# ikramanop/aligner

Hardware: AMD Instinct MI355X
Metric: GCUPS (DP cell updates/s), fill + traceback, inputs resident in HBM (higher is better)
Workload: dtype int32; 1 GPU; C5: 100000 protein pairs, lengths iid U[200,2000], core local (SimpleLocalAligner), BLOSUM62, del 11 / ext 2, seed 0xA11C0005; pairs=100000, cells=121325988939, pairs_ok_rank0=100000, pairs_repaired_or_refilled_rank0=65570

## Files before the change

### aligner_amd/csrc/aln_device.h

```cpp
#pragma once
#include <stdint.h>

#include "../../include/aligner_hip.h"

#ifndef ALN_FULL_R
#define ALN_FULL_R 8
#endif
#define ALN_STRIP_ROWS (64 * ALN_FULL_R)
#define ALN_LAYOUT_SKEW 0u
#define ALN_LAYOUT_ROWMAJOR 1u
#define ALN_LAYOUT_UNIFORM 2u
#define ALN_LAYOUT_UBATCH 3u

struct PairDesc {
    uint64_t q_off, t_off;
    uint32_t N, M;
    uint64_t dir_off;
    uint64_t tb_off;
    uint64_t tag_off;
    uint64_t h_off;
    int32_t status;
    uint32_t layout;
};
#define ALN_PRE_EMPTY_OK (-1)
// ... 85 lines not shown
#define ALN_COOP_ABORTS 6
#define ALN_COOP_SCANS 7
#define ALN_COOP_ULOG 32
#define ALN_COOP_CTL_WORDS 256u

struct SingleArgs {
    const uint8_t *seqs;
    PairDesc *descs;
    uint32_t pair;
    uint8_t *dirs;
    aln_pair_result *results;
    uint32_t *granules;
    uint64_t gstride;
    uint8_t *advice, *zrow;
    int32_t *cand;
    uint32_t *ctrl;
    const void *matrix;
    uint32_t rows, cols;
    double del, ext;
    int32_t semantics;
    uint32_t R, ns, pass, max_passes;
    uint32_t hazard;
    uint32_t store_dirs;
    uint32_t test_drop;
    int *ckpt;
    uint32_t *rgranules;
    int32_t *rcand;
    uint32_t rep_S, rep_K;
    uint32_t mode;
};

#define ALN_CK_SLOTS 7
#define ALN_CK_LAST 1024u
#define ALN_CASCADE_ROWS 3u
#define ALN_CK_FIRST 16u

struct TraceArgs {
    const uint8_t *seqs;
    const PairDesc *descs;
    uint32_t n_pairs;
    const uint8_t *dirs;
    aln_pair_result *results;
    uint8_t *tb;
    uint8_t *tags;
    int32_t semantics;
    uint8_t blank;
    uint8_t pwm;
    uint32_t *walked;
    uint32_t epoch;
    const uint32_t *doneq;
    uint32_t *head;
    uint32_t n_order;
    uint64_t wait_ticks;
};

struct WgArgs {
    const uint8_t *seqs;
    PairDesc *descs;
    uint32_t pair;
    uint8_t *dirs;
    aln_pair_result *results;
    const void *matrix;
    uint32_t rows, cols;
    double del, ext;
    int32_t semantics;
    uint32_t R, ns;
    uint32_t max_passes;
    uint32_t store_dirs;
    uint8_t *scratch;
    void *hmat;
    uint32_t pwm;
};
#define ALN_WG_RING 256u
__host__ __device__ inline uint32_t aln_wg_lds_bytes(uint32_t rows, uint32_t cols, uint32_t sc_size, uint32_t ns, uint32_t N)
{
    return ((rows * cols * sc_size + 15u) & ~15u) + ns * ALN_WG_RING * sc_size + 3u * ((N + 66u + 15u) & ~15u) + 64u * 4u + ns * 32u +
           (N <= 2048u ? (((N + 66u) * sc_size + 15u) & ~15u) : 0u);
}
#define ALN_QRING_BYTES 192u
#define ALN_BRING_BYTES 272u
#define ALN_FEED_BYTES (ALN_QRING_BYTES + ALN_BRING_BYTES)
__host__ __device__ inline uint32_t aln_fast_lds_bytes(uint32_t rows, uint32_t cols, uint32_t prof_stride, uint32_t feed_bytes)
{
    const uint32_t s_bytes = (rows * cols * 4u + 15u) & ~15u;
    return prof_stride == 0u ? s_bytes : s_bytes + 4u * prof_stride + 4u * feed_bytes;
}

struct TraceSingleArgs {
    const uint8_t *seqs;
    const PairDesc *descs;
    uint32_t pair;
    const uint8_t *dirs;
    aln_pair_result *results;
    uint8_t *tb;
    uint8_t *tags;
    int32_t semantics;
    uint32_t R, ns;
    uint4 *map;
    uint4 *seg;
    uint32_t pwm;
};

__host__ __device__ constexpr inline uint32_t aln_spb(uint32_t R) { return R >= 5 ? 2u : R >= 3 ? 4u : 16u / R; }
__host__ __device__ inline int aln_tag_to_dir(int t) { return t == 3 ? 3 : 2 - t; }
__host__ __device__ inline int aln_dir_to_tag(int d) { return d == 3 ? 3 : 2 - d; }
__host__ __device__ inline uint32_t aln_dir_bitpos(uint32_t k, uint32_t r, uint32_t lane, uint32_t N, int R)
// ... 42 lines not shown
```

### aligner_amd/csrc/aln_host.hip

```cpp
#include <hip/hip_runtime.h>

#include <algorithm>
#include <atomic>
#include <cmath>
#include <condition_variable>
#include <cstdio>
#include <cstdlib>
#include <cstring>
#include <deque>
#include <memory>
#include <mutex>
#include <numeric>
#include <string>
#include <chrono>
#include <thread>
#include <vector>

#include "aln_device.h"
#include "aln_loop_rules.h"
#include "aln_plan_rules.h"
#include "aln_scheme_rules.h"
#include "aln_seqset_rules.h"
#include "aln_shuffle_rules.h"

// ... 40 lines not shown
    template <class T> T *as() const { return reinterpret_cast<T *>(p); }
};
static int dev_ensure(DevBuf &b, size_t bytes, bool slack)
{
    bytes = std::max<size_t>(bytes, 256);
    if (b.cap >= bytes) return ALN_OK;
    if (b.p) { (void)hipFree(b.p); b.p = nullptr; b.cap = 0; }
    size_t want = slack ? bytes + bytes / 8 : bytes;
    hipError_t e = hipMalloc(&b.p, want);
    if (e != hipSuccess && want != bytes) { want = bytes; e = hipMalloc(&b.p, want); }
    if (e != hipSuccess) { b.p = nullptr; return fail(e, "hipMalloc"); }
    b.cap = want;
    return ALN_OK;
}
static void dev_free(DevBuf &b)
{
    if (b.p) (void)hipFree(b.p);
    b.p = nullptr; b.cap = 0;
}
struct PinBuf {
    void *p = nullptr;
    size_t cap = 0;
    template <class T> T *as() const { return reinterpret_cast<T *>(p); }
};
static int pin_ensure(PinBuf &b, size_t bytes)
{
    bytes = std::max<size_t>(bytes, 4096);
    if (b.cap >= bytes) return ALN_OK;
    if (b.p) { (void)hipHostFree(b.p); b.p = nullptr; b.cap = 0; }
    const size_t want = bytes + bytes / 4;
    hipError_t e = hipHostMalloc(&b.p, want, hipHostMallocDefault);
    if (e != hipSuccess) { b.p = nullptr; return fail(e, "hipHostMalloc"); }
    b.cap = want;
    return ALN_OK;
}
static void pin_free(PinBuf &b)
{
    if (b.p) (void)hipHostFree(b.p);
    b.p = nullptr; b.cap = 0;
}

struct Slot {
    bool pooled = true;
    DevBuf seqs, descs, order, counter, walked, dirs, results, tb, tags, scratch, matrix, pwm_words, hmat;
    DevBuf granules, advice1, cand, ctrl, tbmap, unpack, repair, coop;
    DevBuf shuffle;
    PinBuf h_meta;
    PinBuf h_in, h_out;
    hipStream_t stream = nullptr;
    hipStream_t tb_stream = nullptr;
    hipEvent_t ev_fork = nullptr, ev_join = nullptr, ev_done = nullptr, ev_fill = nullptr;
    uint32_t epoch = 0;
    bool walked_clean = false;
    uint32_t salt = 0;
    bool scratch_clean = false;
};

struct DevCtx {
    int device = 0;
    int cus = 0;
    size_t hbm = 0;
    char name[128] = {0};
    std::mutex mu;
    std::condition_variable cv;
    Slot *slots[ALN_POOL_SLOTS] = {nullptr};
    bool busy[ALN_POOL_SLOTS] = {false};
};

struct aln_ctx {
    std::vector<DevCtx *> devs;
    std::atomic<uint32_t> turn{0};
    DevCtx *next_device() { return devs[turn.fetch_add(1, std::memory_order_relaxed) % devs.size()]; }
};

static int slot_init(Slot &s)
{
    if (!s.stream) HIPCHK(hipStreamCreateWithFlags(&s.stream, hipStreamNonBlocking));
    if (!s.ev_done) HIPCHK(hipEventCreateWithFlags(&s.ev_done, hipEventDisableTiming));
    if (!s.ev_fill) HIPCHK(hipEventCreateWithFlags(&s.ev_fill, hipEventDisableTiming));
    return ALN_OK;
}
static void slot_destroy(Slot *s)
{
    if (!s) return;
    DevBuf *d[] = {&s->seqs, &s->descs, &s->order, &s->counter, &s->walked, &s->dirs, &s->results, &s->tb, &s->tags, &s->scratch,
                   &s->matrix, &s->pwm_words, &s->hmat, &s->granules, &s->advice1, &s->cand, &s->ctrl, &s->tbmap, &s->unpack, &s->repair, &s->coop,
                   &s->shuffle};
    for (DevBuf *b : d) dev_free(*b);
    pin_free(s->h_meta); pin_free(s->h_in); pin_free(s->h_out);
    if (s->ev_fork) (void)hipEventDestroy(s->ev_fork);
    if (s->ev_join) (void)hipEventDestroy(s->ev_join);
    if (s->ev_done) (void)hipEventDestroy(s->ev_done);
    if (s->ev_fill) (void)hipEventDestroy(s->ev_fill);
    if (s->tb_stream) (void)hipStreamDestroy(s->tb_stream);
    if (s->stream) (void)hipStreamDestroy(s->stream);
    delete s;
}

static int pool_lease(DevCtx *ctx, int want, Slot **out)
{
    std::unique_lock<std::mutex> lk(ctx->mu);
    int got = 0;
    for (;;) {
        for (int i = 0; i < ALN_POOL_SLOTS && got < want; ++i)
            if (!ctx->busy[i]) {
                if (!ctx->slots[i]) ctx->slots[i] = new Slot();
// ... 454 lines not shown
    const uint64_t adv_bytes = ((uint64_t)max_len + 66 + 63) & ~63ull;
    k.cascade_rows = (c.fast && c.semantics == ALN_CORE_LOCAL && c.p.del != c.p.ext) ? ALN_CASCADE_ROWS : (c.fast ? 2u : 1u);
    const uint64_t ck_bytes = c.fast ? (uint64_t)ALN_CK_SLOTS * 18 * 64 * 4 : 0;
    const uint64_t zrow_bytes = std::max<uint64_t>(adv_bytes, ((c.fast ? 8ull : 4ull) * (((uint64_t)max_len + 63) / 2 + 8) + 63) & ~63ull);
    k.zrow_bytes = (uint32_t)zrow_bytes;
    const uint64_t row1_bytes = c.fast ? 0 : brow_bytes + adv_bytes;
    k.scratch_stride = (uint64_t)k.cascade_rows * brow_bytes + adv_bytes + zrow_bytes + ck_bytes + row1_bytes;
    k.lds_bytes = c.pair_matrices ? aln_pairset_lds_bytes(rows, cols) : (uint32_t)(((uint64_t)rows * cols * (c.is_int ? 4 : 8) + 15) & ~15ull);
    k.prof_stride = 0;
    if (c.fast && !pwm) { k.prof_stride = cols * 64u * ALN_FULL_R; k.lds_bytes = aln_fast_lds_bytes(rows, cols, k.prof_stride, ALN_FEED_BYTES); }
    k.duo_qo = 0;
    if (c.fast && !pwm && c.semantics == ALN_CORE_GLOBAL && !k.coop && !k.coop_lean && !k.overlap && !getenv("ALN_NO_DUO") &&
        k.n_small > (uint64_t)ctx->cus * 12u) {
        uint32_t max_rows = 0, max_cols = 0;
        for (size_t j = 0; j < k.n_small; ++j) { const PairDesc &d = k.descs[k.order[j]]; max_rows = std::max(max_rows, d.M); max_cols = std::max(max_cols, d.N); }
        const uint32_t qo = (max_cols + 136u + 7u) & ~7u;
        const uint32_t rmax = (max_rows + 31u) / 32u, rp = rmax > 4u ? 8u : rmax > 2u ? 4u : std::max(rmax, 1u);
        const uint32_t prof = cols * 64u * rp;
        const uint32_t lds = (uint32_t)(((uint64_t)rows * cols * 4 + 15) & ~15ull) + 4u * (prof + 4u * qo);
        if (max_rows <= 256u && max_cols <= 1024u && lds <= 52u * 1024u) {
            k.duo_qo = qo;
            k.prof_stride = prof;
            k.lds_bytes = lds;
            const uint32_t items = (uint32_t)((k.n_small + 1) / 2);
            k.grid = std::max(1u, std::min((items + 3u) / 4u, (uint32_t)ctx->cus * 3u));
        }
    }
    return ALN_OK;
}

struct Need {
    uint64_t seq_span = 0, n = 0, dir_bytes = 0, tb_bytes = 0, tag_bytes = 0, scratch = 0, coop = 0;
};

static int slot_ensure(Slot &s, const Call &c, const Chunk &k, const Need *need = nullptr, bool small_meta = false)
{
    int st;
    const bool sl = s.pooled;
#define ENS(buf, bytes) if ((st = dev_ensure(s.buf, (bytes), sl)) != ALN_OK) return st
    if (need) {
        ENS(seqs, need->seq_span + 64);
        ENS(descs, need->n * sizeof(PairDesc));
        ENS(order, need->n * sizeof(uint32_t));
        ENS(results, need->n * sizeof(aln_pair_result));
        ENS(dirs, need->dir_bytes);
        ENS(tb, need->tb_bytes);
        ENS(tags, need->tag_bytes);
        ENS(scratch, need->scratch);
        if (need->coop) ENS(coop, need->coop);
    }
    ENS(seqs, k.seq_span + 64);
    ENS(descs, k.n * sizeof(PairDesc));
    ENS(order, k.n * sizeof(uint32_t));
    ENS(counter, k.counter_bytes);
    if (k.coop) ENS(coop, k.coop_bytes);
    if (k.overlap) {
        const size_t before = s.walked.cap;
        ENS(walked, 4ull * k.n);
        if (s.walked.cap != before) s.walked_clean = false;
        if (!s.tb_stream) HIPCHK(hipStreamCreateWithFlags(&s.tb_stream, hipStreamNonBlocking));
        if (!s.ev_fork) HIPCHK(hipEventCreateWithFlags(&s.ev_fork, hipEventDisableTiming));
        if (!s.ev_join) HIPCHK(hipEventCreateWithFlags(&s.ev_join, hipEventDisableTiming));
    }
    ENS(dirs, k.dir_bytes);
    ENS(results, k.n * sizeof(aln_pair_result));
    ENS(tb, k.tb_bytes);
    ENS(tags, k.tag_bytes);
    {
        const size_t before = s.scratch.cap;
        const void *before_p = s.scratch.p;
        ENS(scratch, std::max<uint64_t>((uint64_t)k.grid * 4 * k.scratch_stride, k.wg_pairs.empty() ? 0 : ((uint64_t)k.max_len + 66) * 8));
        if (s.scratch.cap != before || s.scratch.p != before_p) s.scratch_clean = false;
    }
    if (!k.wg_pairs.empty()) ENS(tbmap, k.tbmap_entries * 16);
    ENS(matrix, (uint64_t)c.rows * c.cols * (c.is_int ? 4 : 8));
    if (c.pwm && c.fast) ENS(pwm_words, (uint64_t)c.cols * 4);
    if (c.want_h) ENS(hmat, k.hmat_elems * (c.is_int ? 4 : 8));
    if (!k.single_pairs.empty()) {
        ENS(granules, k.granule_bytes);
        ENS(advice1, 2ull * single_advice_bytes(k.single_max_n));
        ENS(cand, 16ull * (k.single_max_n + 64));
        ENS(ctrl, 256);
        ENS(tbmap, k.tbmap_entries * 16);
        ENS(repair, 8ull * (k.granule_stride_max * 4 + 18 * 64 * 4 + 32) + 256);
    }
#undef ENS
    const size_t meta = (small_meta ? 0 : std::max<size_t>(k.n, need ? need->n : 0) * (sizeof(PairDesc) + 4)) + (size_t)c.rows * c.cols * 8 + (size_t)c.cols * 4 + 256;
    if ((st = pin_ensure(s.h_meta, meta)) != ALN_OK) return st;
    if (!small_meta && !k.seq_direct && (st = pin_ensure(s.h_in, k.seq_span + 64)) != ALN_OK) return st;
    return slot_init(s);
}

static int upload_matrix(Slot &s, const Call &c, uint8_t *m, hipStream_t st)
{
    size_t o = 0;
    const size_t nm = c.md.size();
    if (c.is_int) {
        int32_t *mi = reinterpret_cast<int32_t *>(m + o);
        for (size_t i = 0; i < nm; ++i) mi[i] = (int32_t)c.md[i];
        HIPCHK(hipMemcpyAsync(s.matrix.p, mi, nm * 4, hipMemcpyHostToDevice, st));
    } else {
        memcpy(m + o, c.md.data(), nm * 8);
        HIPCHK(hipMemcpyAsync(s.matrix.p, m + o, nm * 8, hipMemcpyHostToDevice, st));
    }
    o += nm * 8;
    if (c.pwm && c.fast) {
        uint32_t *words = reinterpret_cast<uint32_t *>(m + o);
        for (uint32_t x = 0; x < c.cols; ++x) {
            uint32_t wv = 0;
            for (uint32_t r = 0; r < 4; ++r) wv |= ((uint32_t)(int32_t)(4 * (int32_t)c.md[(size_t)r * c.cols + x] - 2) & 0xffu) << (8 * r);
            words[x] = wv;
        }
        HIPCHK(hipMemcpyAsync(s.pwm_words.p, words, (size_t)c.cols * 4, hipMemcpyHostToDevice, st));
    }
    return ALN_OK;
}

static int slot_upload(Slot &s, const Call &c, const Chunk &k, const uint8_t *seqs, const uint64_t *q_off, const uint64_t *q_len,
                       const uint64_t *t_off, const uint64_t *t_len, hipStream_t st, bool staged = false, bool seqs_there = false)
{
    uint8_t *m = s.h_meta.as<uint8_t>();
    size_t o = 0;
    if (k.n) {
        memcpy(m + o, k.descs.data(), k.n * sizeof(PairDesc));
        HIPCHK(hipMemcpyAsync(s.descs.p, m + o, k.n * sizeof(PairDesc), hipMemcpyHostToDevice, st));
        o += k.n * sizeof(PairDesc);
        if (!k.order.empty()) {
            memcpy(m + o, k.order.data(), k.order.size() * 4);
            HIPCHK(hipMemcpyAsync(s.order.p, m + o, k.order.size() * 4, hipMemcpyHostToDevice, st));
        }
        o += k.n * 4;
    }
    o = (o + 15) & ~(size_t)15;
    int e = upload_matrix(s, c, m + o, st);
    if (e != ALN_OK) return e;
    if (k.seq_span && !seqs_there) {
        if (k.seq_direct) {
            HIPCHK(hipMemcpyAsync(s.seqs.p, seqs + k.seq_lo, k.seq_span, hipMemcpyHostToDevice, st));
        } else {
            uint8_t *h = s.h_in.as<uint8_t>();
            for (size_t i = 0; i < k.n && !staged; ++i) {
                const size_t g = k.first + i;
                if (!c.pwm && q_len[g]) memcpy(h + k.descs[i].q_off, seqs + q_off[g], q_len[g]);
                if (t_len[g]) memcpy(h + k.descs[i].t_off, seqs + t_off[g], t_len[g]);
            }
            HIPCHK(hipMemcpyAsync(s.seqs.p, h, k.seq_span, hipMemcpyHostToDevice, st));
        }
    }
    return ALN_OK;
}

static int slot_launch(DevCtx *ctx, Slot &s, const Call &c, const Chunk &k, hipStream_t st, hipEvent_t *ev, uint32_t *fill_launches,
                       hipEvent_t fill_after = nullptr)
{
    if (fill_launches) *fill_launches = 0;
    if (k.n == 0) return ALN_OK;
    if (k.n_small) HIPCHK(hipMemsetAsync(s.counter.p, 0, k.counter_bytes, st));
    if (k.n_small && k.coop) HIPCHK(hipMemsetAsync(s.coop.p, 0, k.coop_bytes, st));
    if (k.n_small && c.fast) {
        s.salt = (s.salt + 1u) & 0x3ffu;
        if (!s.scratch_clean || s.salt == 0u) { HIPCHK(hipMemsetAsync(s.scratch.p, 0, s.scratch.cap, st)); s.scratch_clean = true; }
    }
    if (!k.single_pairs.empty())
        aln_launch_validate(s.seqs.as<uint8_t>(), s.descs.as<PairDesc>(), (uint32_t)k.n, c.rows, c.cols, c.pwm ? 1 : 0, st);
    FillArgs fa{};
    fa.seqs = s.seqs.as<uint8_t>(); fa.descs = s.descs.as<PairDesc>(); fa.order = s.order.as<uint32_t>(); fa.n_pairs = (uint32_t)k.n_small;
    fa.counter = s.counter.as<uint32_t>(); fa.dirs = s.dirs.as<uint8_t>(); fa.results = s.results.as<aln_pair_result>();
    fa.scratch = s.scratch.as<uint8_t>(); fa.scratch_stride = k.scratch_stride; fa.max_len = k.max_len; fa.zrow_bytes = k.zrow_bytes;
    fa.cascade_rows = k.cascade_rows;
    fa.matrix = s.matrix.p; fa.rows = c.rows; fa.cols = c.cols; fa.prof_stride = k.prof_stride;
    fa.del = c.p.del; fa.ext = c.p.ext; fa.semantics = c.semantics;
    fa.max_passes = c.p.max_passes; fa.force_serial = c.p.force_serial;
    fa.no_repair = getenv("ALN_NO_REPAIR") ? 1u : 0u;
    fa.f64_old = getenv("ALN_F64_OLD") ? 1u : 0u;
    if (c.pair_matrices) { fa.matrix = c.pair_matrices + k.first * ((size_t)c.rows * c.cols); fa.pair_matrices = 1u; fa.f64_old = 0u; }
    fa.max_cells = k.max_cells;
    fa.store_dirs = c.store_dirs ? 1u : 0u;
    fa.pwm = c.pwm ? 1u : 0u;
    fa.pwm_words = s.pwm_words.as<uint32_t>();
    fa.hmat = c.want_h ? s.hmat.p : nullptr; fa.blank = c.p.blank_code;
    fa.n_descs = (uint32_t)k.n;
    { const char *e = getenv("ALN_BACK_WAVES"); fa.back_waves = (e && atoi(e) && k.grid == (uint32_t)ctx->cus * 3u && k.n_small >= 2ull * k.grid * 4u) ? 1u : 0u; }
    fa.coop = k.coop ? s.coop.as<uint32_t>() : nullptr; fa.coop_waves = k.grid * 4u; fa.coop_tail = k.coop_tail; fa.salt = s.salt;
    { const char *e = getenv("ALN_COOP_LINGER"); fa.coop_linger = e ? (uint32_t)atoi(e) : (k.coop_linger ? 1u : 0u); }
    { const char *e = getenv("ALN_COOP_DEBUG"); fa.coop_debug = e ? (uint32_t)atoi(e) : 0u; }
    { const char *e = getenv("ALN_FAIR"); fa.fair = e ? (uint32_t)atoi(e) : 0u; }
    { const char *e = getenv("ALN_CK_LAST"); fa.ck_last = (e && atoi(e) == 512) ? 512u : ALN_CK_LAST; }
    fa.duo_qo = k.duo_qo;
    fa.claim = 1;
    if (c.fast && !k.coop && !k.coop_lean && !fa.back_waves && k.max_cells <= (1ull << 18) && k.n_small != 0) {
        const double per_wave = (double)(k.duo_qo ? (k.n_small + 1) / 2 : k.n_small) / ((double)std::min(k.grid, (uint32_t)ctx->cus * 3u) * 4.0);
        fa.claim = (per_wave >= 3.2 && per_wave < 12.0) ? 2u : 1u;
    }
    if (const char *e = getenv("ALN_CLAIM")) fa.claim = (uint32_t)std::max(1, std::min(8, atoi(e)));
    if (fill_after) HIPCHK(hipStreamWaitEvent(st, fill_after, 0));
    if (ev) HIPCHK(hipEventRecord(ev[0], st));
    uint32_t launches = 0;
    TraceArgs ta{};
    ta.seqs = s.seqs.as<uint8_t>(); ta.descs = s.descs.as<PairDesc>(); ta.n_pairs = (uint32_t)k.n; ta.dirs = s.dirs.as<uint8_t>();
    ta.results = s.results.as<aln_pair_result>(); ta.tb = s.tb.as<uint8_t>(); ta.tags = s.tags.as<uint8_t>();
    ta.semantics = c.semantics; ta.blank = c.p.blank_code; ta.pwm = c.pwm ? 1 : 0;
    const bool overlap = k.overlap;
    if (overlap) {
        if (!s.walked_clean) { HIPCHK(hipMemsetAsync(s.walked.p, 0, s.walked.cap, st)); s.walked_clean = true; s.epoch = 0; }
        fa.doneq = s.counter.as<uint32_t>() + 64;
        ta.walked = s.walked.as<uint32_t>(); ta.epoch = ++s.epoch; ta.n_order = (uint32_t)k.n_small;
        ta.doneq = s.counter.as<uint32_t>() + 64; ta.head = s.counter.as<uint32_t>() + 2; ta.wait_ticks = 50000000ull;
        if (const char *w = getenv("ALN_TB_WAIT_US")) ta.wait_ticks = 100ull * strtoull(w, nullptr, 10);
        HIPCHK(hipEventRecord(s.ev_fork, st));
    }
    if (k.n_small) {
        aln_launch_fill(&fa, c.is_int ? 1 : 0, c.fast ? 1 : 0, k.grid, k.lds_bytes, st);
        HIPCHK(hipGetLastError());
        launches = 1;
    }
    if (overlap) {
        HIPCHK(hipStreamWaitEvent(s.tb_stream, s.ev_fork, 0));
        aln_launch_traceback_overlap(&ta, k.tb_waves, s.tb_stream);
        HIPCHK(hipGetLastError());
        HIPCHK(hipEventRecord(s.ev_join, s.tb_stream));
    }
    for (size_t j = 0; j < k.single_pairs.size(); ++j) {
        const PairDesc &d = k.descs[k.single_pairs[j]];
        SingleArgs sa{};
        sa.seqs = s.seqs.as<uint8_t>(); sa.descs = s.descs.as<PairDesc>(); sa.pair = k.single_pairs[j]; sa.dirs = s.dirs.as<uint8_t>();
        sa.results = s.results.as<aln_pair_result>(); sa.granules = s.granules.as<uint32_t>();
        sa.gstride = ((uint64_t)d.N + 64 + 63) & ~63ull;
        sa.advice = s.advice1.as<uint8_t>(); sa.zrow = s.advice1.as<uint8_t>() + single_advice_bytes(k.single_max_n);
        sa.cand = s.cand.as<int32_t>(); sa.ctrl = s.ctrl.as<uint32_t>(); sa.matrix = s.matrix.p;
        sa.rows = c.rows; sa.cols = c.cols; sa.del = c.p.del; sa.ext = c.p.ext;
        sa.semantics = c.semantics; sa.R = k.single_r[j];
        sa.ns = (d.M + 64 * sa.R - 1) / (64 * sa.R);
        sa.hazard = (sa.semantics == ALN_CORE_LOCAL && sa.del != sa.ext && d.N >= 2) ? 1u : 0u;
        sa.store_dirs = c.store_dirs ? 1u : 0u;
        { const char *td = getenv("ALN_TEST_DROP_STRIP"); sa.test_drop = td ? (uint32_t)atoi(td) : 0u; }
        if (getenv("ALN_TEST_FAIL_REPAIR")) sa.test_drop = 0xffffffffu;
        sa.max_passes = sa.hazard ? std::min<uint32_t>(c.p.max_passes ? c.p.max_passes : 4u, 12u) : 1u;
        sa.rep_S = 0; sa.rep_K = 0; sa.mode = 0;
        {
            const uint32_t S = sa.R >= 2 ? 4u : 8u, K = 256u;
            if (sa.hazard && !getenv("ALN_NO_SINGLE_REPAIR") && sa.R <= 2 && sa.ns > S && d.N >= K + 64u * S + 128u) { sa.rep_S = S; sa.rep_K = K; }
            uint8_t *rb = s.repair.as<uint8_t>();
            sa.rgranules = reinterpret_cast<uint32_t *>(rb);
            sa.ckpt = reinterpret_cast<int *>(rb + 8ull * k.granule_stride_max * 4);
            sa.rcand = reinterpret_cast<int32_t *>(rb + 8ull * k.granule_stride_max * 4 + 8ull * 18 * 64 * 4);
        }
        aln_launch_single_init(&sa, (uint32_t)single_advice_bytes(d.N), st);
        HIPCHK(hipMemsetAsync(s.granules.p, 0, (size_t)sa.ns * sa.gstride * 4, st));
        for (uint32_t pass = 0; pass < sa.max_passes; ++pass) {
            sa.pass = pass;
            aln_launch_single(&sa, d.N, pass + 1 == sa.max_passes ? 1 : 0, st);
            launches++;
            if (pass == 0 && sa.rep_S) aln_launch_single_repair(&sa, d.N, st);
        }
        HIPCHK(hipGetLastError());
    }
    for (size_t j = 0; j < k.wg_pairs.size(); ++j) {
        const PairDesc &d = k.descs[k.wg_pairs[j]];
        WgArgs wa{};
        wa.seqs = s.seqs.as<uint8_t>(); wa.descs = s.descs.as<PairDesc>(); wa.pair = k.wg_pairs[j]; wa.dirs = s.dirs.as<uint8_t>();
        wa.results = s.results.as<aln_pair_result>(); wa.matrix = s.matrix.p; wa.rows = c.rows; wa.cols = c.cols;
        wa.del = c.p.del; wa.ext = c.p.ext; wa.semantics = c.semantics; wa.R = k.wg_r[j]; wa.ns = (d.M + 64 * wa.R - 1) / (64 * wa.R);
        wa.max_passes = c.p.max_passes; wa.store_dirs = c.store_dirs ? 1u : 0u; wa.scratch = s.scratch.as<uint8_t>();
        wa.hmat = c.want_h ? s.hmat.p : nullptr;
        wa.pwm = c.pwm ? 1u : 0u;
        aln_launch_wgpipe(&wa, c.is_int ? 1 : 0, aln_wg_lds_bytes(c.rows, c.cols, c.is_int ? 4u : 8u, wa.ns, d.N), st);
        launches++;
        HIPCHK(hipGetLastError());
    }
    if (ev) HIPCHK(hipEventRecord(ev[1], st));
    if (s.ev_fill) HIPCHK(hipEventRecord(s.ev_fill, st));
    if (c.want_tb && c.store_dirs) {
        if (overlap) HIPCHK(hipStreamWaitEvent(st, s.ev_join, 0));
        const bool batch_tb = k.n_small != 0 || c.semantics == ALN_CORE_LOCAL || !k.wg_pairs.empty();
        if (batch_tb) {
            bool wave_walk = k.n <= 2048 || (k.n < 4096 && k.max_len >= 1024);
            if (const char *e = getenv("ALN_TB_WAVE")) wave_walk = atoi(e) != 0;
            if (wave_walk) aln_launch_traceback_wave(&ta, st);
            else aln_launch_traceback(&ta, st);
        }
        for (size_t j = 0; j < k.single_pairs.size(); ++j) {
            const PairDesc &d = k.descs[k.single_pairs[j]];
            TraceSingleArgs tsa{};
            tsa.seqs = s.seqs.as<uint8_t>(); tsa.descs = s.descs.as<PairDesc>(); tsa.pair = k.single_pairs[j]; tsa.dirs = s.dirs.as<uint8_t>();
            tsa.results = s.results.as<aln_pair_result>(); tsa.tb = s.tb.as<uint8_t>(); tsa.tags = s.tags.as<uint8_t>();
            tsa.semantics = c.semantics;
            tsa.R = k.single_r[j]; tsa.ns = (d.M + 64 * tsa.R - 1) / (64 * tsa.R);
            tsa.map = s.tbmap.as<uint4>(); tsa.seg = s.tbmap.as<uint4>() + (uint64_t)tsa.ns * (d.N + 1);
            aln_launch_traceback_single(&tsa, d.N, st);
            aln_launch_traceback_expand_single(&ta, tsa.pair, st);
        }
        for (size_t j = 0; j < k.wg_pairs.size(); ++j) {
            const PairDesc &d = k.descs[k.wg_pairs[j]];
            TraceSingleArgs tsa{};
            tsa.seqs = s.seqs.as<uint8_t>(); tsa.descs = s.descs.as<PairDesc>(); tsa.pair = k.wg_pairs[j]; tsa.dirs = s.dirs.as<uint8_t>();
            tsa.results = s.results.as<aln_pair_result>(); tsa.tb = s.tb.as<uint8_t>(); tsa.tags = s.tags.as<uint8_t>();
            tsa.semantics = c.semantics;
            tsa.R = k.wg_r[j]; tsa.ns = (d.M + 64 * tsa.R - 1) / (64 * tsa.R);
            tsa.map = s.tbmap.as<uint4>(); tsa.seg = s.tbmap.as<uint4>() + (uint64_t)tsa.ns * (d.N + 1);
            tsa.pwm = c.pwm ? 1u : 0u;
            aln_launch_traceback_single(&tsa, d.N, st);
            aln_launch_traceback_expand_single(&ta, tsa.pair, st);
        }
        if (batch_tb) aln_launch_traceback_expand(&ta, st);
        HIPCHK(hipGetLastError());
    }
    if (c.unscale != 1.0) { aln_launch_scale_results(s.results.as<aln_pair_result>(), (uint32_t)k.n, c.unscale, st); HIPCHK(hipGetLastError()); }
    if (ev) HIPCHK(hipEventRecord(ev[2], st));
    if (fill_launches) *fill_launches = launches;
    return ALN_OK;
}

static void coop_stats_slot(Slot &s, const Chunk &k)
{
    if (k.coop && getenv("ALN_COOP_STATS")) {
        uint32_t w[256] = {0};
        if (hipMemcpy(w, s.coop.p, sizeof w, hipMemcpyDeviceToHost) == hipSuccess) {
            if (w[14]) {
                fprintf(stderr, "coop: %u strips left rows without their tag; the first: N %u, strip %u of %u, R %u, own %u, open %u; columns (tag found):", w[14], w[16], (w[15] >> 4), w[17] >> 8,
                        w[15] & 15u, w[17] & 1u, (w[17] >> 1) & 1u);
                for (int i = 0; i < 40 && w[128 + i]; ++i) fprintf(stderr, " %u(%#x)", w[128 + i], w[192 + i]);
                fprintf(stderr, "\n");
            }
            fprintf(stderr, "coop: urgent passes %u, unclaimed strips now %d urgent %d lazy, finished %u, strips helped %u, scans %u, aborted passes %u, spins waiting for strips to finish %u; "
                    "strips that gave up waiting for the row above %u, owners that gave up waiting for a strip %u, bottom-row records not found %u, pair granules not found %u\n",
                    w[ALN_COOP_ULOGW], (int)w[ALN_COOP_UOPEN], (int)w[ALN_COOP_LOPEN], w[ALN_COOP_FINISHED], w[ALN_COOP_HELPED], w[ALN_COOP_SCANS], w[ALN_COOP_ABORTS], w[9],
                    w[10], w[11], w[12], w[13]);
        }
    }
}
static int slot_download(Slot &s, const Call &c, const Chunk &k, hipStream_t st, aln_pair_result *results, uint8_t *tb_buf,
                         const uint64_t *tb_off)
{
    if (k.n == 0) return ALN_OK;
    HIPCHK(hipMemcpyAsync(results + k.first, s.results.p, k.n * sizeof(aln_pair_result), hipMemcpyDeviceToHost, st));
    const bool want = tb_buf && tb_off && c.store_dirs && c.want_tb && k.tb_bytes;
    bool direct = want;
    if (want) {
        const uint64_t base = tb_off[k.first];
        for (size_t i = 0; i < k.n && direct; ++i) direct = tb_off[k.first + i] - base == k.descs[i].tb_off && tb_off[k.first + i] >= base;
        if (direct) HIPCHK(hipMemcpyAsync(tb_buf + base, s.tb.p, k.tb_bytes, hipMemcpyDeviceToHost, st));
        else {
            int e = pin_ensure(s.h_out, k.tb_bytes);
            if (e != ALN_OK) return e;
            HIPCHK(hipMemcpyAsync(s.h_out.p, s.tb.p, k.tb_bytes, hipMemcpyDeviceToHost, st));
        }
    }
    HIPCHK(hipStreamSynchronize(st));
    coop_stats_slot(s, k);
    if (want && !direct) {
        const uint8_t *h = s.h_out.as<uint8_t>();
        for (size_t i = 0; i < k.n; ++i) {
            const PairDesc &d = k.descs[i];
            const aln_pair_result &r = results[k.first + i];
            if (r.status != ALN_OK) continue;
            const uint64_t cap = (uint64_t)d.N + d.M + 2;
            uint8_t *dst = tb_buf + tb_off[k.first + i];
            if (c.pwm) {
// ... 2426 lines not shown
```

### aligner_amd/csrc/aln_kernels.hip

```cpp
#include <hip/hip_runtime.h>
#include <float.h>
#include <limits.h>
#include <math.h>

#include "aln_device.h"

#define ALN_PART_GENERIC 1
#define ALN_PART_FAST_CL 2
#define ALN_PART_FAST_REST 4
#define ALN_PART_FAST_CL_SOLO 32
#define ALN_PART_FAST_REST_SOLO 64
#define ALN_PART_SINGLE 8
#define ALN_PART_TB 16
#ifndef ALN_TU
#define ALN_TU 127
#endif

namespace {

constexpr int D_TOP = 0, D_LEFT = 1, D_DIAG = 2, D_BEG = 3;

template <typename SC> struct ScOps;

template <> struct ScOps<int> {
// ... 2167 lines not shown
                uint32_t dq = (uint32_t)__builtin_amdgcn_readlane((int)qrow, (int)lane) + 1u - qr;
                if (!have || dq > 2u) {
                    const int t = iy - (int)(lane_id * R + R - 1u);
                    const int kj = (cxm - (t > 0 ? t : 0)) + (int)lane_id - (int)(R >> 1);
                    qrow = (uint32_t)(kj > 0 ? kj : 0) >> qsh;
                    if (lane_id == lane) qrow = qr;
                    const bool on = lane_id <= lane;
                    wa = wb = wc = make_uint4(0, 0, 0, 0);
                    if (on && qrow + 1u < nq) wa = wq[((size_t)(qrow + 1u) << 6) + lane_id];
                    if (on && qrow < nq) wb = wq[((size_t)qrow << 6) + lane_id];
                    if (on && qrow >= 1u) wc = wq[((size_t)(qrow - 1u) << 6) + lane_id];
                    have = true;
                    dq = 1u;
                }
                const int li = (int)lane;
                if (dq == 0u) { q0 = __builtin_amdgcn_readlane((int)wa.x, li); q1 = __builtin_amdgcn_readlane((int)wa.y, li); q2 = __builtin_amdgcn_readlane((int)wa.z, li); q3 = __builtin_amdgcn_readlane((int)wa.w, li); }
                else if (dq == 1u) { q0 = __builtin_amdgcn_readlane((int)wb.x, li); q1 = __builtin_amdgcn_readlane((int)wb.y, li); q2 = __builtin_amdgcn_readlane((int)wb.z, li); q3 = __builtin_amdgcn_readlane((int)wb.w, li); }
                else { q0 = __builtin_amdgcn_readlane((int)wc.x, li); q1 = __builtin_amdgcn_readlane((int)wc.y, li); q2 = __builtin_amdgcn_readlane((int)wc.z, li); q3 = __builtin_amdgcn_readlane((int)wc.w, li); }
                cur_lane = lane; cur_q = qr;
                asm volatile("" : "+s"(cur_lane), "+s"(cur_q));
            }
            const uint32_t lend = lane + Nm1;
            const uint32_t m = min(k | bmask, lend) - k;
            const uint32_t j = (k >> lgS) & 3u;
            const uint64_t half = (j & 2u) ? (((uint64_t)q3 << 32) | q2) : (((uint64_t)q1 << 32) | q0);
            const uint32_t tag = (uint32_t)(half >> (32u * (j & 1u) + 32u - 2u * R * (m + 1u) + 2u * r)) & 3u;
            if (tag == 3u) {
                cy = (uint32_t)(iy + 1) + sv.y0; cx = (uint32_t)(cxm + 1);
                break;
            }
            tagv = (uint32_t)__builtin_amdgcn_update_dpp((int)tag, (int)tagv, 0x138, 0xf, 0xf, false);
            ++len;
            if ((len & 63u) == 0u) ops[len - 1u - lane_id] = (uint8_t)tagv;
            iy -= (tag != 1u); cxm -= (tag != 2u);
        }
    }
    if (lane_id < (len & 63u)) ops[len - 1u - lane_id] = (uint8_t)tagv;
    if (global) {
        if (cy == 0 && cx != 0) { for (uint32_t i = lane_id; i < cx; i += 64u) ops[len + i] = 1; len += cx; cx = 0; }
        else if (cx == 0 && cy != 0) { for (uint32_t i = lane_id; i < cy; i += 64u) ops[len + i] = 2; len += cy; cy = 0; }
    }
    if (lane_id == 0) {
        res.start_y = cy; res.start_x = cx;
        res.aln_len = len + (a.pwm ? 0u : 1u);
    }
}
extern "C" __global__ __launch_bounds__(256) void aln_traceback_wave_kernel(TraceArgs a)
{
    const uint32_t pair = uni32(blockIdx.x * 4u + (threadIdx.x >> 6));
    if (pair >= a.n_pairs) return;
    if (a.walked && uni32(a.walked[pair]) == a.epoch) return;
    tb_walk_pair_wave(a, pair);
}
extern "C" __global__ __attribute__((amdgpu_flat_work_group_size(64, 64), amdgpu_num_vgpr(16))) void aln_traceback_overlap_kernel(TraceArgs a)
{
    __builtin_amdgcn_s_setprio(3);
    for (;;) {
        uint32_t base = 0;
        if (threadIdx.x == 0) base = __hip_atomic_fetch_add(a.head, 64u, __ATOMIC_RELAXED, __HIP_MEMORY_SCOPE_AGENT);
        base = (uint32_t)__builtin_amdgcn_readfirstlane((int)base);
        if (base >= a.n_order) return;
        const uint32_t my = base + threadIdx.x;
        uint32_t v = 0;
        const uint64_t t0 = wall_clock64();
        for (;;) {
            if (my < a.n_order && v == 0) v = __hip_atomic_load(a.doneq + my, __ATOMIC_RELAXED, __HIP_MEMORY_SCOPE_SYSTEM);
            if (__all(my >= a.n_order || v != 0)) break;
            __builtin_amdgcn_s_sleep(127);
            if (wall_clock64() - t0 > a.wait_ticks) return;
        }
        __atomic_thread_fence(__ATOMIC_ACQUIRE);
        if (my < a.n_order) {
            tb_walk_pair(a, v - 1u);
            a.walked[v - 1u] = a.epoch;
        }
    }
}
extern "C" __global__ __launch_bounds__(64) void aln_delay_kernel(uint32_t ticks)
{
    const uint64_t t0 = wall_clock64();
    while (wall_clock64() - t0 < ticks) __builtin_amdgcn_s_sleep(64);
}

struct StripWindow {
    const uint32_t *wbase;
    const uint32_t *lds;
    uint32_t q_lo, q_n;
};
__device__ __forceinline__ StripWindow stage_window(const uint32_t *wbase, uint32_t *lds, uint32_t lds_quads, uint32_t k_hi,
                                                    uint32_t lgR)
{
    StripWindow w;
    const uint32_t sh = 4u - lgR;
    const uint32_t q_hi = k_hi >> (sh + 2);
    w.wbase = wbase; w.lds = lds;
    w.q_n = min(lds_quads, q_hi + 1u);
    w.q_lo = q_hi + 1u - w.q_n;
    const uint4 *src = reinterpret_cast<const uint4 *>(wbase) + (size_t)w.q_lo * 64u;
    uint4 *dst = reinterpret_cast<uint4 *>(lds);
    const uint32_t n = w.q_n * 64u;
    uint4 v[12];
#pragma unroll
    for (uint32_t j = 0; j < 12; ++j) {
        const uint32_t i = threadIdx.x + j * 256u;
        if (i < n) v[j] = src[i];
    }
#pragma unroll
    for (uint32_t j = 0; j < 12; ++j) {
        const uint32_t i = threadIdx.x + j * 256u;
        if (i < n) dst[i] = v[j];
    }
    __syncthreads();
    return w;
}

template <class Fetch>
__device__ __forceinline__ bool walk_in_strip(Fetch fetch, uint32_t y0, uint32_t lgR, uint32_t N, bool global,
                                              uint32_t &cy, uint32_t &cx, uint32_t &steps, uint8_t *ops,
                                              uint32_t cap = 0xffffffffu, bool *gave_up = nullptr)
{
    const uint32_t R = 1u << lgR, sh = 4u - lgR;
    uint32_t y = cy, x = cx, n = steps;
    const uint32_t n_stop = cap == 0xffffffffu ? cap : steps + cap;
    bool beginning = false;
    bool go = (y > y0 && x != 0);
    while (go) {
        const uint32_t i = y - 1 - y0;
// ... 150 lines not shown
        return word;
    };
    if (threadIdx.x == 0) walk_in_strip(fetch, y0, lgR, d.N, global, cy, cx, steps, ops);
}

extern "C" __global__ __launch_bounds__(1024) void aln_tb_single_expand_kernel(TraceArgs a, uint32_t pair)
{
    __shared__ uint32_t wsum_y[16], wsum_x[16];
    const PairDesc &d = a.descs[pair];
    const aln_pair_result &res = a.results[pair];
    if (res.status != ALN_OK || (d.layout & 0xffu) != ALN_LAYOUT_UNIFORM) return;
    const uint32_t tid = threadIdx.x, lane = tid & 63u, wave = tid >> 6;
    const uint8_t *__restrict__ q = a.seqs + d.q_off;
    const uint8_t *__restrict__ t = a.seqs + d.t_off;
    const uint32_t cap = d.N + d.M + 2;
    uint8_t *__restrict__ qa = a.tb + d.tb_off;
    uint8_t *__restrict__ ta = qa + (a.pwm ? 4ull : 1ull) * cap;
    uint32_t *__restrict__ numbered = reinterpret_cast<uint32_t *>(qa);
    const uint8_t *__restrict__ ops = a.tags + d.tag_off;
    const uint32_t len = res.aln_len - (a.pwm ? 0u : 1u);
    const uint32_t per = (len + 1023u) / 1024u;
    const uint32_t lo = min(len, tid * per), hi = min(len, lo + per);
    uint32_t dy = 0, dx = 0;
    for (uint32_t j = lo; j < hi; ++j) {
        const uint32_t tag = ops[len - 1 - j];
        dx += (tag != 2u); dy += (tag != 1u);
    }
    uint32_t sy = dy, sx = dx;
#pragma unroll
    for (int m = 1; m < 64; m <<= 1) {
        const uint32_t oy = (uint32_t)__shfl_up((int)sy, m), ox = (uint32_t)__shfl_up((int)sx, m);
        if ((int)lane >= m) { sy += oy; sx += ox; }
    }
    if (lane == 63) { wsum_y[wave] = sy; wsum_x[wave] = sx; }
    __syncthreads();
    uint32_t by = 0, bx = 0;
    for (uint32_t wv = 0; wv < wave; ++wv) { by += wsum_y[wv]; bx += wsum_x[wv]; }
    uint32_t py = res.start_y + by + sy - dy, px = res.start_x + bx + sx - dx;
    for (uint32_t j = lo; j < hi; ++j) {
        const uint32_t tag = ops[len - 1 - j];
        px += (tag != 2u); py += (tag != 1u);
        if (a.pwm) numbered[j] = (tag == 2u) ? 0u : px;
        else qa[j] = (tag == 2u) ? a.blank : q[px - 1];
        ta[j] = (tag == 1u) ? a.blank : t[py - 1];
    }
    if (tid == 0 && !a.pwm) {
        qa[len] = q[res.end_x - 1];
        ta[len] = t[res.end_y - 1];
    }
}

extern "C" __global__ __attribute__((amdgpu_flat_work_group_size(256, 256), amdgpu_num_vgpr(16))) void aln_traceback_expand_kernel(TraceArgs a)
{
    const uint32_t pair = blockIdx.x * (blockDim.x >> 6) + (threadIdx.x >> 6);
    if (pair >= a.n_pairs) return;
    constexpr int G = 2;
    const int lane = threadIdx.x & 63;
    const PairDesc &d = a.descs[pair];
    const aln_pair_result &res = a.results[pair];
    if (res.status != ALN_OK) return;
    if ((d.layout & 0xffu) == ALN_LAYOUT_UNIFORM) return;
    const uint8_t *__restrict__ q = a.seqs + d.q_off;
    const uint8_t *__restrict__ t = a.seqs + d.t_off;
    const uint32_t cap = d.N + d.M + 2;
    uint8_t *__restrict__ qa = a.tb + d.tb_off;
    uint8_t *__restrict__ ta = qa + (a.pwm ? 4ull : 1ull) * cap;
    const uint8_t *__restrict__ ops = a.tags + d.tag_off;
    uint32_t *__restrict__ numbered = reinterpret_cast<uint32_t *>(qa);
    const uint32_t len = res.aln_len - (a.pwm ? 0u : 1u);
    uint32_t base_y = (uint32_t)__builtin_amdgcn_readfirstlane((int)res.start_y);
    uint32_t base_x = (uint32_t)__builtin_amdgcn_readfirstlane((int)res.start_x);
    for (uint32_t j0 = 0; j0 < len; j0 += 64u * G) {
        uint32_t tag[G], px[G], py[G];
#pragma unroll
        for (int u = 0; u < G; ++u) {
            const uint32_t j = j0 + 64u * u + (uint32_t)lane;
            tag[u] = (j < len) ? (uint32_t)ops[len - 1 - j] : 3u;
        }
#pragma unroll
        for (int u = 0; u < G; ++u) {
            const bool fx = (tag[u] != 2u) && (tag[u] != 3u), fy = (tag[u] != 1u) && (tag[u] != 3u);
            const uint64_t bx = __ballot(fx), by = __ballot(fy);
            px[u] = base_x + __builtin_amdgcn_mbcnt_hi((uint32_t)(bx >> 32), __builtin_amdgcn_mbcnt_lo((uint32_t)bx, 0u)) + (fx ? 1u : 0u);
            py[u] = base_y + __builtin_amdgcn_mbcnt_hi((uint32_t)(by >> 32), __builtin_amdgcn_mbcnt_lo((uint32_t)by, 0u)) + (fy ? 1u : 0u);
            base_x += (uint32_t)__popcll(bx); base_y += (uint32_t)__popcll(by);
        }
        uint32_t qv[G], tv[G];
#pragma unroll
        for (int u = 0; u < G; ++u) {
            qv[u] = (tag[u] == 2u || tag[u] == 3u) ? (uint32_t)a.blank : (a.pwm ? px[u] : (uint32_t)q[px[u] - 1]);
            tv[u] = (tag[u] == 1u || tag[u] == 3u) ? (uint32_t)a.blank : (uint32_t)t[py[u] - 1];
        }
#pragma unroll
        for (int u = 0; u < G; ++u) {
            const uint32_t j = j0 + 64u * u + (uint32_t)lane;
            if (j < len) {
                if (a.pwm) numbered[j] = (tag[u] == 2u) ? 0u : px[u];
                else qa[j] = (uint8_t)qv[u];
                ta[j] = (uint8_t)tv[u];
            }
        }
    }
    if (lane == 0 && !a.pwm) {
        qa[len] = q[res.end_x - 1];
        ta[len] = t[res.end_y - 1];
    }
}

// ... 460 lines not shown
```

Measured before the change: 2916 GCUPS.

## Expand alignments inside overlap traceback kernel and fold counter clear into expand

The overlapped traceback kernel now also expands each walked pair into aligned query/target strings, one lane per pair, for pairs finished before a configurable tail, and marks them in an extra expanded array so the later batch expand kernel skips them. Behind an env flag, the expand kernel also zeroes the counter buffer so the next launch can skip its memset. The aim is to move expansion work off the critical path into the overlap with fill. The cost is per-lane serial expansion with uncoalesced byte stores, more work in the 16-VGPR overlap kernel, and a doubled walked allocation.

```diff
diff --git a/aligner_amd/csrc/aln_device.h b/aligner_amd/csrc/aln_device.h
--- a/aligner_amd/csrc/aln_device.h
+++ b/aligner_amd/csrc/aln_device.h
@@ -161,6 +161,10 @@
     uint32_t *head;
     uint32_t n_order;
     uint64_t wait_ticks;
+    uint32_t *expanded;
+    uint32_t expand_until;
+    uint32_t *clear;
+    uint32_t clear_words;
 };
 
 struct WgArgs {
diff --git a/aligner_amd/csrc/aln_host.hip b/aligner_amd/csrc/aln_host.hip
--- a/aligner_amd/csrc/aln_host.hip
+++ b/aligner_amd/csrc/aln_host.hip
@@ -116,6 +116,8 @@
     hipEvent_t ev_fork = nullptr, ev_join = nullptr, ev_done = nullptr, ev_fill = nullptr;
     uint32_t epoch = 0;
     bool walked_clean = false;
+    size_t counter_zero_bytes = 0;
+    hipStream_t counter_zero_stream = nullptr;
     uint32_t salt = 0;
     bool scratch_clean = false;
 };
@@ -676,11 +678,16 @@
     ENS(seqs, k.seq_span + 64);
     ENS(descs, k.n * sizeof(PairDesc));
     ENS(order, k.n * sizeof(uint32_t));
-    ENS(counter, k.counter_bytes);
+    {
+        const size_t before = s.counter.cap;
+        const void *before_p = s.counter.p;
+        ENS(counter, k.counter_bytes);
+        if (s.counter.cap != before || s.counter.p != before_p) s.counter_zero_bytes = 0;
+    }
     if (k.coop) ENS(coop, k.coop_bytes);
     if (k.overlap) {
         const size_t before = s.walked.cap;
-        ENS(walked, 4ull * k.n);
+        ENS(walked, 8ull * k.n);
         if (s.walked.cap != before) s.walked_clean = false;
         if (!s.tb_stream) HIPCHK(hipStreamCreateWithFlags(&s.tb_stream, hipStreamNonBlocking));
         if (!s.ev_fork) HIPCHK(hipEventCreateWithFlags(&s.ev_fork, hipEventDisableTiming));
@@ -774,12 +781,21 @@
     return ALN_OK;
 }
 
+static bool tb_short_tail()
+{
+    const char *e = getenv("ALN_TB_SHORT_TAIL");
+    return e && atoi(e) != 0;
+}
+
 static int slot_launch(DevCtx *ctx, Slot &s, const Call &c, const Chunk &k, hipStream_t st, hipEvent_t *ev, uint32_t *fill_launches,
                        hipEvent_t fill_after = nullptr)
 {
     if (fill_launches) *fill_launches = 0;
     if (k.n == 0) return ALN_OK;
-    if (k.n_small) HIPCHK(hipMemsetAsync(s.counter.p, 0, k.counter_bytes, st));
+    if (k.n_small) {
+        if (s.counter_zero_bytes < k.counter_bytes || s.counter_zero_stream != st) HIPCHK(hipMemsetAsync(s.counter.p, 0, k.counter_bytes, st));
+        s.counter_zero_bytes = 0;
+    }
     if (k.n_small && k.coop) HIPCHK(hipMemsetAsync(s.coop.p, 0, k.coop_bytes, st));
     if (k.n_small && c.fast) {
         s.salt = (s.salt + 1u) & 0x3ffu;
@@ -831,6 +847,9 @@
         ta.walked = s.walked.as<uint32_t>(); ta.epoch = ++s.epoch; ta.n_order = (uint32_t)k.n_small;
         ta.doneq = s.counter.as<uint32_t>() + 64; ta.head = s.counter.as<uint32_t>() + 2; ta.wait_ticks = 50000000ull;
         if (const char *w = getenv("ALN_TB_WAIT_US")) ta.wait_ticks = 100ull * strtoull(w, nullptr, 10);
+        uint64_t tail = tb_short_tail() ? std::min<uint64_t>(8192u, k.n_small / 8) : k.n_small;
+        if (const char *e = getenv("ALN_TB_EXPAND_TAIL")) tail = std::min<uint64_t>(strtoull(e, nullptr, 10), k.n_small);
+        ta.expanded = s.walked.as<uint32_t>() + k.n; ta.expand_until = (uint32_t)(k.n_small - tail);
         HIPCHK(hipEventRecord(s.ev_fork, st));
     }
     if (k.n_small) {
@@ -926,8 +945,11 @@
             aln_launch_traceback_single(&tsa, d.N, st);
             aln_launch_traceback_expand_single(&ta, tsa.pair, st);
         }
+        const bool clears = overlap && batch_tb && tb_short_tail() && k.counter_bytes / 4 <= 64ull * k.n;
+        if (clears) { ta.clear = s.counter.as<uint32_t>(); ta.clear_words = (uint32_t)(k.counter_bytes / 4); }
         if (batch_tb) aln_launch_traceback_expand(&ta, st);
         HIPCHK(hipGetLastError());
+        if (clears) { s.counter_zero_bytes = k.counter_bytes; s.counter_zero_stream = st; }
     }
     if (c.unscale != 1.0) { aln_launch_scale_results(s.results.as<aln_pair_result>(), (uint32_t)k.n, c.unscale, st); HIPCHK(hipGetLastError()); }
     if (ev) HIPCHK(hipEventRecord(ev[2], st));
diff --git a/aligner_amd/csrc/aln_kernels.hip b/aligner_amd/csrc/aln_kernels.hip
--- a/aligner_amd/csrc/aln_kernels.hip
+++ b/aligner_amd/csrc/aln_kernels.hip
@@ -2243,6 +2243,53 @@
     if (a.walked && uni32(a.walked[pair]) == a.epoch) return;
     tb_walk_pair_wave(a, pair);
 }
+__device__ __forceinline__ void tb_expand_pair_lane(const TraceArgs &a, uint32_t pair)
+{
+    constexpr uint32_t G = 4;
+    const PairDesc &d = a.descs[pair];
+    const aln_pair_result &res = a.results[pair];
+    if (res.status != ALN_OK) return;
+    if ((d.layout & 0xffu) == ALN_LAYOUT_UNIFORM) return;
+    const uint8_t *__restrict__ q = a.seqs + d.q_off;
+    const uint8_t *__restrict__ t = a.seqs + d.t_off;
+    const uint32_t cap = d.N + d.M + 2;
+    uint8_t *__restrict__ qa = a.tb + d.tb_off;
+    uint8_t *__restrict__ ta = qa + (a.pwm ? 4ull : 1ull) * cap;
+    uint32_t *__restrict__ numbered = reinterpret_cast<uint32_t *>(qa);
+    const uint32_t len = res.aln_len - (a.pwm ? 0u : 1u);
+    const uint8_t *last = a.tags + d.tag_off + len;
+    uint32_t px = res.start_x, py = res.start_y;
+    uint32_t j = 0;
+    for (; j + G <= len; j += G) {
+        uint32_t tag[G], qv[G], tv[G];
+#pragma unroll
+        for (uint32_t u = 0; u < G; ++u) tag[u] = last[-1 - (int64_t)(j + u)];
+#pragma unroll
+        for (uint32_t u = 0; u < G; ++u) {
+            px += (tag[u] != 2u); py += (tag[u] != 1u);
+            const uint32_t qr = a.pwm ? px : (uint32_t)q[max(px, 1u) - 1u], tr = (uint32_t)t[max(py, 1u) - 1u];
+            qv[u] = (tag[u] == 2u) ? (a.pwm ? 0u : (uint32_t)a.blank) : qr;
+            tv[u] = (tag[u] == 1u) ? (uint32_t)a.blank : tr;
+        }
+#pragma unroll
+        for (uint32_t u = 0; u < G; ++u) {
+            if (a.pwm) numbered[j + u] = qv[u];
+            else qa[j + u] = (uint8_t)qv[u];
+            ta[j + u] = (uint8_t)tv[u];
+        }
+    }
+    for (; j < len; ++j) {
+        const uint32_t tag = last[-1 - (int64_t)j];
+        px += (tag != 2u); py += (tag != 1u);
+        if (a.pwm) numbered[j] = (tag == 2u) ? 0u : px;
+        else qa[j] = (tag == 2u) ? a.blank : q[px - 1];
+        ta[j] = (tag == 1u) ? a.blank : t[py - 1];
+    }
+    if (!a.pwm) {
+        qa[len] = q[res.end_x - 1];
+        ta[len] = t[res.end_y - 1];
+    }
+}
 extern "C" __global__ __attribute__((amdgpu_flat_work_group_size(64, 64), amdgpu_num_vgpr(16))) void aln_traceback_overlap_kernel(TraceArgs a)
 {
     __builtin_amdgcn_s_setprio(3);
@@ -2261,9 +2308,14 @@
             if (wall_clock64() - t0 > a.wait_ticks) return;
         }
         __atomic_thread_fence(__ATOMIC_ACQUIRE);
+        const bool expand = a.expanded != nullptr && min(base + 64u, a.n_order) <= a.expand_until;
         if (my < a.n_order) {
             tb_walk_pair(a, v - 1u);
             a.walked[v - 1u] = a.epoch;
+            if (expand) {
+                tb_expand_pair_lane(a, v - 1u);
+                a.expanded[v - 1u] = a.epoch;
+            }
         }
     }
 }
@@ -2520,8 +2572,13 @@
 
 extern "C" __global__ __attribute__((amdgpu_flat_work_group_size(256, 256), amdgpu_num_vgpr(16))) void aln_traceback_expand_kernel(TraceArgs a)
 {
+    if (a.clear) {
+        const uint32_t i = blockIdx.x * blockDim.x + threadIdx.x;
+        if (i < a.clear_words) a.clear[i] = 0u;
+    }
     const uint32_t pair = blockIdx.x * (blockDim.x >> 6) + (threadIdx.x >> 6);
     if (pair >= a.n_pairs) return;
+    if (a.expanded && uni32(a.expanded[pair]) == a.epoch) return;
     constexpr int G = 2;
     const int lane = threadIdx.x & 63;
     const PairDesc &d = a.descs[pair];
```

New measurement: 2917 GCUPS (median of 4 runs). No clear change (+0.1%).
